# HiLab-git/FPL-plus

Hardware: NVIDIA B200
Metric: train_voxels_per_s (higher is better)
Workload: dtype bf16

## Files before the change

fpl-plus_b200/csrc/convt_tc.cu:

```cuda
#include "common.cuh"
#include "tc_ptx.cuh"
#include "../../include/fplplus_b200.h"

namespace {

constexpr int kTH = 16, kTW = 8;
constexpr int kPlane = kTH * kTW * 16;
constexpr int kThreadsT = 192;
constexpr int kMaxStagesT = 8;

__device__ __forceinline__ void tma_load_4d(void* dst, const CUtensorMap* map, uint64_t* bar, int c0, int c1, int c2, int c3) {
    asm volatile(
        "cp.async.bulk.tensor.4d.shared::cluster.global.tile.mbarrier::complete_tx::bytes [%0], [%1, {%3, %4, %5, %6}], [%2];"
        ::"r"(smem_u32(dst)), "l"(map), "r"(smem_u32(bar)), "r"(c0), "r"(c1), "r"(c2), "r"(c3)
        : "memory");
}

struct CtParams {
    const __nv_bfloat16* image;
    const float* bias;
    bf16x8* out;
    int out_c8tot, out_c8off;
    int a_c8tot, a_c8off;
    int N, D, H, W;
// ... 202 lines not shown
        int ci, co, tap;
        if (mode == 0) { ci = k; tap = nn / cout; co = nn - tap * cout; }
        else { tap = k / cout; co = k - tap * cout; ci = nn; }
        image[i] = __float2bfloat16_rn(w[((int64_t)ci * cout + co) * ntaps + tap]);
    }
}

CUresult encode_4d(EncodeTiledFn encode, CUtensorMap* map, const void* base, int64_t planes, int h, int w, int box_c8,
                   int stride) {
    cuuint64_t gdim[4] = {8, (cuuint64_t)w, (cuuint64_t)h, (cuuint64_t)planes};
    cuuint64_t gstr[3] = {16, (cuuint64_t)w * 16, (cuuint64_t)h * w * 16};
    cuuint32_t box[4] = {8, (cuuint32_t)(kTW * stride), (cuuint32_t)(kTH * stride), (cuuint32_t)box_c8};
    cuuint32_t estr[4] = {1, (cuuint32_t)stride, (cuuint32_t)stride, 1};
    return encode(map, CU_TENSOR_MAP_DATA_TYPE_BFLOAT16, 4, const_cast<void*>(base), gdim, gstr, box, estr,
                  CU_TENSOR_MAP_INTERLEAVE_NONE, CU_TENSOR_MAP_SWIZZLE_NONE, CU_TENSOR_MAP_L2_PROMOTION_L2_128B,
                  CU_TENSOR_MAP_FLOAT_OOB_FILL_NONE);
}

struct CtwParams {
    float* dw;
    int N, D, H, W, cin, cout, kd2, ntaps;
    int x_c8tot, x_c8off, dy_c8tot, dy_c8off;
    int mgroups, m, nb, mtiles, nchunks;
    int x_bytes, dy_tile_bytes, stage_bytes, stages, tmem_cols;
    int tiles_h, tiles_w, tiles_total, split;
    int tapmajor;
};

__global__ void __launch_bounds__(kThreadsT) convt_wgrad_tc_kernel(const __grid_constant__ CUtensorMap xmap,
                                                                  const __grid_constant__ CUtensorMap dymap, CtwParams P) {
    extern __shared__ uint8_t smem_raw[];
    uint8_t* smem = reinterpret_cast<uint8_t*>((reinterpret_cast<uintptr_t>(smem_raw) + 1023) & ~uintptr_t(1023));
    uint64_t* bars = reinterpret_cast<uint64_t*>(smem);
    uint64_t* full_bar = bars;
    uint64_t* empty_bar = bars + kMaxStagesT;
    uint64_t* done_bar = bars + 2 * kMaxStagesT;
    uint32_t* tmem_slot = reinterpret_cast<uint32_t*>(bars + 2 * kMaxStagesT + 1);
    uint8_t* ring = smem + 256;

    const int warp = threadIdx.x >> 5, lane = threadIdx.x & 31;
    int b = blockIdx.x;
    const int slice = b % P.split; b /= P.split;
    const int nc = b % P.nchunks;
    const int mt = b / P.nchunks;
    const int tile_begin = (int)(((int64_t)P.tiles_total * slice) / P.split);
    const int tile_end = (int)(((int64_t)P.tiles_total * (slice + 1)) / P.split);
    const int Do = P.D * P.kd2;

    if (warp == 0 && lane == 0) {
        asm volatile("prefetch.tensormap [%0];" ::"l"(&xmap) : "memory");
        asm volatile("prefetch.tensormap [%0];" ::"l"(&dymap) : "memory");
        for (int s = 0; s < P.stages; ++s) { mbar_init(&full_bar[s], 1); mbar_init(&empty_bar[s], 1); }
        mbar_init(done_bar, 1);
        fence_barrier_init();
    }
    if (warp == 1) tmem_alloc(tmem_slot, (uint32_t)P.tmem_cols);
    FPL_PDL_WAIT();
    tc_fence_before();
    __syncthreads();
    tc_fence_after();
    const uint32_t tmem_base = *tmem_slot;

    if (warp == 0) {
        if (lane == 0) {
            int stage = 0; uint32_t phase = 0;
            for (int t = tile_begin; t < tile_end; ++t) {
                int r = t;
                const int tw = r % P.tiles_w; r /= P.tiles_w;
                const int th = r % P.tiles_h; r /= P.tiles_h;
                const int d = r % P.D;
                const int n = r / P.D;
                mbar_wait(&empty_bar[stage], phase ^ 1);
                uint8_t* x_dst = ring + (size_t)stage * P.stage_bytes;
                mbar_expect_tx(&full_bar[stage], (uint32_t)(P.x_bytes + P.ntaps * P.dy_tile_bytes));
                tma_load_4d(x_dst, &xmap, &full_bar[stage], 0, tw * kTW, th * kTH,
                            (n * P.D + d) * P.x_c8tot + P.x_c8off + mt * P.mgroups);
                for (int tap = 0; tap < P.ntaps; ++tap) {
                    const int a = P.kd2 == 2 ? tap >> 2 : 0, bb = (tap >> 1) & 1, c = tap & 1;
                    tma_load_4d(x_dst + P.x_bytes + (size_t)tap * P.dy_tile_bytes, &dymap, &full_bar[stage], 0,
                                2 * tw * kTW + c, 2 * th * kTH + bb,
                                (n * Do + d * P.kd2 + a) * P.dy_c8tot + P.dy_c8off + nc * (P.nb / 8));
                }
                if (++stage == P.stages) { stage = 0; phase ^= 1; }
            }
        }
    } else if (warp == 1) {
        const uint32_t idesc = (1u << 4) | (1u << 7) | (1u << 10) | (1u << 15) | (1u << 16) |
                               ((uint32_t)(P.nb >> 3) << 17) | ((uint32_t)(P.m >> 4) << 24);
        const uint64_t hi = make_desc(0, kTW * 16, kPlane);
        const uint32_t ring_u = smem_u32(ring);
        const bool leader = elect_one();
        int stage = 0; uint32_t phase = 0;
        uint32_t accumulate = 0;
        for (int t = tile_begin; t < tile_end; ++t) {
            mbar_wait(&full_bar[stage], phase);
            tc_fence_after();
            const uint32_t x_base = (ring_u + (uint32_t)stage * (uint32_t)P.stage_bytes) >> 4;
            const uint32_t dy_base = x_base + ((uint32_t)P.x_bytes >> 4);
            uint64_t adesc = hi + (uint64_t)x_base, b_hp = hi + (uint64_t)dy_base;
            const uint64_t dy_tile16 = (uint64_t)((uint32_t)P.dy_tile_bytes >> 4);
            for (int hp = 0; hp < kTH / 2; ++hp, adesc += 2 * kTW * 16 / 16, b_hp += 2 * kTW * 16 / 16) {
                uint64_t bdesc = b_hp;
                uint32_t d_tap = tmem_base;
                for (int tap = 0; tap < P.ntaps; ++tap, bdesc += dy_tile16, d_tap += (uint32_t)P.nb) {
                    if (leader) umma_bf16(d_tap, adesc, bdesc, idesc, accumulate);
                }
                accumulate = 1;
            }
            if (leader) umma_commit(&empty_bar[stage]);
            __syncwarp();
            if (++stage == P.stages) { stage = 0; phase ^= 1; }
        }
        if (leader) umma_commit(done_bar);
        __syncwarp();
        FPL_PDL_TRIGGER();
    } else if (tile_end > tile_begin) {
        const int quarter = warp & 3;
        mbar_wait(done_bar, 0);
        tc_fence_after();
        const int tlane = quarter * 32 + lane;
        int row = P.m == 128 ? tlane : ((lane < 16) ? quarter * 16 + lane : -1);
        const bool valid = row >= 0 && row < P.mgroups * 8 && (mt * P.mgroups * 8 + row) < P.cin;
        const int ci = mt * P.mgroups * 8 + row;
        for (int tap = 0; tap < P.ntaps; ++tap) {
            for (int c0 = 0; c0 < P.nb; c0 += 16) {
                uint32_t r[16];
                tmem_ld16(tmem_base + ((uint32_t)(quarter * 32) << 16) + (uint32_t)(tap * P.nb + c0), r);
                tmem_ld_wait();
                if (valid) {
#pragma unroll
                    for (int i = 0; i < 16; ++i) {
                        const int co = nc * P.nb + c0 + i;
                        if (P.tapmajor) atomicAdd(P.dw + ((int64_t)tap * P.cout + co) * P.cin + ci, __uint_as_float(r[i]));
                        else atomicAdd(P.dw + ((int64_t)ci * P.cout + co) * P.ntaps + tap, __uint_as_float(r[i]));
                    }
                }
            }
        }
    }
    tc_fence_before();
    __syncthreads();
    if (warp == 1) {
        tc_fence_after();
        tmem_dealloc(tmem_base, (uint32_t)P.tmem_cols);
    }
}

}

extern "C" int64_t fpl_convt_weight_image_bytes(int cin, int cout, int kd2) {
    return (int64_t)cin * cout * 4 * kd2 * 2;
}

extern "C" int fpl_convt_prep_weight(const float* w, int cin, int cout, int kd2, int mode, void* image, void* stream) {
    FPL_REQUIRE(kd2 == 1 || kd2 == 2, "fpl_convt_prep_weight: kd2=%d must be 1 or 2", kd2);
    const int ntaps = 4 * kd2;
    CtCfg c;
    const int kdim = mode == 0 ? cin : ntaps * cout, ndim = mode == 0 ? ntaps * cout : cin;
    FPL_REQUIRE(make_ct_cfg(kdim, ndim, mode == 0 ? cin : cout, c), "fpl_convt_prep_weight: unsupported channels (%d -> %d)", cin, cout);
    const int total = kdim * ndim;
    int blocks = (total + 255) / 256;
    if (blocks > FPL_NUM_SMS * 4) blocks = FPL_NUM_SMS * 4;
    fpl_launch(convt_prep_kernel, blocks, 256, 0, (cudaStream_t)stream, w, (__nv_bfloat16*)image, cin, cout, ntaps, mode, c.nb, c.kc,
                                                               c.nchunks, total);
    FPL_LAUNCH_CHECK();
    return 0;
}

// ... 75 lines not shown
    int64_t total = (int64_t)P.tiles_h * P.tiles_w * d * n * c.nslices;
    FPL_REQUIRE(total < (1ll << 30), "fpl_convt_k2s2_tc: too many tiles");
    P.total_items = (int)total;
    FPL_CHECK_CUDA(cudaFuncSetAttribute(convt_gemm_tc_kernel, cudaFuncAttributeMaxDynamicSharedMemorySize, c.smem_bytes));
    int grid = FPL_NUM_SMS * 2;
    if (grid > P.total_items) grid = P.total_items;
    fpl_launch(convt_gemm_tc_kernel, grid, kThreadsT, c.smem_bytes, (cudaStream_t)stream, amap, P);
    FPL_LAUNCH_CHECK();
    return 0;
}

extern "C" int fpl_convt_k2s2_fwd_tc(const void* x, int x_c8tot, int x_c8off, const void* image, const float* bias, void* y,
                                     int y_c8tot, int y_c8off, int n, int d, int h, int w, int cin, int cout, int kd2,
                                     void* stream) {
    return convt_gemm_launch(0, x, x_c8tot, x_c8off, image, bias, y, y_c8tot, y_c8off, n, d, h, w, cin, cout, kd2, stream);
}

extern "C" int fpl_convt_k2s2_dgrad_tc(const void* dy, int dy_c8tot, int dy_c8off, const void* image_t, void* dx, int dx_c8tot,
                                       int dx_c8off, int n, int d, int h, int w, int cin, int cout, int kd2, void* stream) {
    return convt_gemm_launch(1, dy, dy_c8tot, dy_c8off, image_t, nullptr, dx, dx_c8tot, dx_c8off, n, d, h, w, cin, cout, kd2,
                             stream);
}

static int convt_wgrad_launch(const void* x, int x_c8tot, int x_c8off, const void* dy, int dy_c8tot, int dy_c8off,
                              float* dw, int n, int d, int h, int w, int cin, int cout, int kd2, void* stream, int tapmajor) {
    FPL_REQUIRE(kd2 == 1 || kd2 == 2, "fpl_convt_k2s2_wgrad_tc: kd2=%d must be 1 or 2", kd2);
    FPL_REQUIRE(cin % 8 == 0 && cout % 16 == 0, "fpl_convt_k2s2_wgrad_tc: unsupported channels (%d -> %d)", cin, cout);
    EncodeTiledFn encode = get_encode_fn();
    FPL_REQUIRE(encode != nullptr, "fpl_convt_k2s2_wgrad_tc: cuTensorMapEncodeTiled not available from the driver");
    CtwParams P;
    P.dw = dw; P.N = n; P.D = d; P.H = h; P.W = w; P.cin = cin; P.cout = cout; P.kd2 = kd2; P.ntaps = 4 * kd2;
    P.x_c8tot = x_c8tot; P.x_c8off = x_c8off; P.dy_c8tot = dy_c8tot; P.dy_c8off = dy_c8off; P.tapmajor = tapmajor;
    const int g_all = cin / 8;
    P.mgroups = g_all < 16 ? g_all : 16;
    FPL_REQUIRE(g_all % P.mgroups == 0, "fpl_convt_k2s2_wgrad_tc: cin=%d not tileable", cin);
    P.mtiles = g_all / P.mgroups;
    P.m = P.mgroups <= 8 ? 64 : 128;
    P.nb = cout % 32 == 0 ? 32 : 16;
    P.x_bytes = P.mgroups * kPlane;
    if (2 * (P.x_bytes + P.ntaps * (P.nb / 8) * kPlane) > 200 * 1024 - (P.m / 8) * kPlane) P.nb = 16;
    P.nchunks = cout / P.nb;
    P.dy_tile_bytes = (P.nb / 8) * kPlane;
    P.stage_bytes = P.x_bytes + P.ntaps * P.dy_tile_bytes;
    P.stages = (200 * 1024 - (P.m / 8) * kPlane) / P.stage_bytes;
    if (P.stages > kMaxStagesT) P.stages = kMaxStagesT;
    FPL_REQUIRE(P.stages >= 2, "fpl_convt_k2s2_wgrad_tc: stage of %d bytes does not fit twice", P.stage_bytes);
    int cols = P.ntaps * P.nb;
    P.tmem_cols = 32;
    while (P.tmem_cols < cols) P.tmem_cols *= 2;
    CUtensorMap xmap, dymap;
    CUresult r = encode_4d(encode, &xmap, x, (int64_t)n * d * x_c8tot, h, w, P.mgroups, 1);
    FPL_REQUIRE(r == CUDA_SUCCESS, "fpl_convt_k2s2_wgrad_tc: tensor map (x) failed (%d)", (int)r);
    r = encode_4d(encode, &dymap, dy, (int64_t)n * d * kd2 * dy_c8tot, 2 * h, 2 * w, P.nb / 8, 2);
    FPL_REQUIRE(r == CUDA_SUCCESS, "fpl_convt_k2s2_wgrad_tc: tensor map (dy) failed (%d)", (int)r);
    P.tiles_h = (h + kTH - 1) / kTH; P.tiles_w = (w + kTW - 1) / kTW;
    int64_t tiles = (int64_t)P.tiles_h * P.tiles_w * d * n;
    FPL_REQUIRE(tiles < (1ll << 30), "fpl_convt_k2s2_wgrad_tc: too many tiles");
    P.tiles_total = (int)tiles;
    const int pairs = P.mtiles * P.nchunks;
    int split = FPL_NUM_SMS / pairs;
    if (split > P.tiles_total / 4) split = P.tiles_total / 4;
    if (split < 1) split = 1;
    P.split = split;
    const int smem_bytes = P.stages * P.stage_bytes + (P.m / 8) * kPlane + 1024 + 256;
    FPL_CHECK_CUDA(cudaFuncSetAttribute(convt_wgrad_tc_kernel, cudaFuncAttributeMaxDynamicSharedMemorySize, smem_bytes));
    fpl_launch(convt_wgrad_tc_kernel, pairs * split, kThreadsT, smem_bytes, (cudaStream_t)stream, xmap, dymap, P);
    FPL_LAUNCH_CHECK();
    return 0;
}

extern "C" int fpl_convt_k2s2_wgrad_tc(const void* x, int x_c8tot, int x_c8off, const void* dy, int dy_c8tot, int dy_c8off,
                                       float* dw, int n, int d, int h, int w, int cin, int cout, int kd2, void* stream) {
    return convt_wgrad_launch(x, x_c8tot, x_c8off, dy, dy_c8tot, dy_c8off, dw, n, d, h, w, cin, cout, kd2, stream, 0);
}

extern "C" int fpl_convt_k2s2_wgrad_tc_tapmajor(const void* x, int x_c8tot, int x_c8off, const void* dy, int dy_c8tot,
                                                int dy_c8off, float* scratch, int n, int d, int h, int w, int cin, int cout,
                                                int kd2, void* stream) {
    return convt_wgrad_launch(x, x_c8tot, x_c8off, dy, dy_c8tot, dy_c8off, scratch, n, d, h, w, cin, cout, kd2, stream, 1);
}
```

fpl-plus_b200/lib.py:

```python
import ctypes
from ctypes import c_char_p, c_double, c_float, c_int, c_int64, c_longlong, c_uint64, c_void_p

from . import build as _build

_P = c_void_p
_I = c_int
_L = c_int64
_F = c_float
_U = c_uint64

_SIGNATURES = {
    "fpl_last_error": (c_char_p, []),
    "fpl_version": (_I, []),
    "fpl_set_sm_budget": (_I, [_I]),
    "fpl_launch_count": (c_longlong, [_I]),
    "fpl_device_is_sm100": (_I, []),
    "fpl_conv3d_weight_image_bytes": (_L, [_I, _I, _I]),
    "fpl_conv3d_prep_weight": (_I, [_P, _I, _I, _I, _I, _P, _P]),
    "fpl_conv3d_prep_weight_batch": (_I, [_I, ctypes.POINTER(c_void_p), ctypes.POINTER(_I), ctypes.POINTER(_I),
                                          ctypes.POINTER(_I), ctypes.POINTER(_I), ctypes.POINTER(c_void_p), _P]),
    "fpl_conv3d_tc": (_I, [_P, _I, _I, _P, _P, _P, _I, _I, _P] + [_I] * 7 + [_P]),
    "fpl_conv3d_dfold_image_bytes": (_L, [_I, _I]),
    "fpl_conv3d_dfold_prep_weight": (_I, [_P, _I, _I, _I, _P, _P]),
    "fpl_conv3d_dfold_prep_weight_batch": (_I, [_I, ctypes.POINTER(c_void_p), ctypes.POINTER(_I), ctypes.POINTER(_I),
# ... 16 lines not shown
    "fpl_maxpool_c8": (_I, [_P, _I, _I, _P, _I, _I, _I] + [_I] * 5 + [_P]),
    "fpl_head_fwd": (_I, [_P, _I, _I, _P, _P, _P] + [_I] * 6 + [_P]),
    "fpl_head_dgrad": (_I, [_P, _P, _P, _I, _I, _P, _I, _I, _P] + [_I] * 6 + [_P]),
    "fpl_upsample2x_c8": (_I, [_P, _I, _I, _P, _I, _I] + [_I] * 6 + [_P]),
    "fpl_upsample2x_c8_bwd": (_I, [_P, _I, _I, _P, _I, _I] + [_I] * 6 + [_P]),
    "fpl_channel_sum_c8": (_I, [_P, _I, _I, _P] + [_I] * 5 + [_P]),
    "fpl_grad_scatter_add": (_I, [_P, _P, _P, _I, _I, _P]),
    "fpl_stem_conv_fwd": (_I, [_P, _P, _P, _P, _I, _I, _P] + [_I] * 7 + [_P]),
    "fpl_stem_conv_wgrad": (_I, [_P, _P, _I, _I, _P] + [_I] * 7 + [_P]),
    "fpl_head_conv_fwd": (_I, [_P, _I, _I, _P, _P, _P] + [_I] * 6 + [_P]),
    "fpl_head_conv_tc": (_I, [_P, _I, _I, _P, _P, _P] + [_I] * 6 + [_P]),
    "fpl_pack_ncdhw_to_c8": (_I, [_P, _I, _P, _I, _I, _I, _P] + [_I] * 4 + [_P]),
    "fpl_head_conv_bwd": (_I, [_P, _I, _I, _P, _P, _P, _I, _I, _P, _P] + [_I] * 6 + [_P]),
    "fpl_convt_k2s2_fwd": (_I, [_P, _I, _I, _P, _P, _P, _I, _I] + [_I] * 7 + [_P]),
    "fpl_convt_k2s2_bwd": (_I, [_P, _I, _I, _P, _P, _I, _I, _P, _I, _I, _P, _P] + [_I] * 7 + [_P]),
    "fpl_convt_weight_image_bytes": (_L, [_I, _I, _I]),
    "fpl_convt_prep_weight": (_I, [_P, _I, _I, _I, _I, _P, _P]),
    "fpl_convt_prep_weight_batch": (_I, [_I, ctypes.POINTER(c_void_p), ctypes.POINTER(_I), ctypes.POINTER(_I),
                                         ctypes.POINTER(_I), ctypes.POINTER(_I), ctypes.POINTER(c_void_p), _P]),
    "fpl_convt_k2s2_fwd_tc": (_I, [_P, _I, _I, _P, _P, _P, _I, _I] + [_I] * 7 + [_P]),
    "fpl_convt_k2s2_dgrad_tc": (_I, [_P, _I, _I, _P, _P, _I, _I] + [_I] * 7 + [_P]),
    "fpl_convt_k2s2_wgrad_tc": (_I, [_P, _I, _I, _P, _I, _I, _P] + [_I] * 7 + [_P]),
    "fpl_convt_k2s2_wgrad_tc_tapmajor": (_I, [_P, _I, _I, _P, _I, _I, _P] + [_I] * 7 + [_P]),
    "fpl_dsbn_finalize": (_I, [_P, _L, _P, _P, _P, _P, _P, _F, _F, _I, _P, _P, _P, _P, _I, _P]),
    "fpl_dsbn_act_fwd": (_I, [_P, _P, _P, _P, _P, _I, _I, _P, _I, _I, _P, _I, _F, _P, _U, _U, _P] + [_I] * 5 + [_P]),
    "fpl_dsbn_bn_act_fwd": (_I, [_P, _P, _L, _P, _P, _P, _P, _P, _F, _F, _I, _P, _P, _P, _P, _P,
                                 _P, _I, _I, _P, _I, _I, _P, _I, _F, _P, _U, _U, _P] + [_I] * 5 + [_P]),
    "fpl_dsbn_act_bwd_apply_fin": (_I, [_P, _P, _I, _I, _P, _I, _I, _P, _I, _P, _P, _P, _P, _P, _F, _P, _U, _U, _P, _P, _I, _P]
                                   + [_I] * 5 + [_P, _P, _P, _P, _P]),
    "fpl_dsbn_act_bwd_reduce": (_I, [_P, _P, _I, _I, _P, _I, _I, _P, _I, _P, _P, _P, _P, _P, _F, _P, _U, _U, _P, _P]
                                + [_I] * 5 + [_P]),
    "fpl_dsbn_act_bwd_apply": (_I, [_P, _P, _I, _I, _P, _I, _I, _P, _I, _P, _P, _P, _P, _P, _F, _P, _U, _U, _P, _P, _I, _P]
                               + [_I] * 5 + [_P]),
    "fpl_dsbn_bwd_finalize": (_I, [_P, _P, _P, _I, _P, _P, _P, _P, _I, _P]),
    "fpl_gather_patches": (_I, [_P, _I, _I, _I, _I, _I, _P, _P, _P, _P]),
    "fpl_gather_patches_norm_workspace_bytes": (_L, [_I] * 5),
    "fpl_gather_patches_norm": (_I, [_P, _I, _I, _I, _I, _I, ctypes.POINTER(_I), ctypes.POINTER(_F), ctypes.POINTER(_F), _P,
                                     _L, _P, _P, _P, _P]),
    "fpl_adam_multi_tensor": (_I, [_P, _I, _P, _I, _P, c_double, c_double, c_double, c_double, c_double, _P, _P]),
    "fpl_adam_chunk_elems": (_I, []),
    "fpl_dice_ce_reduce": (_I, [_P, _P, _P, _P, _I, _I, _L, _P]),
    "fpl_dice_ce_grad": (_I, [_P, _P, _P, _P, _F, _F, _F, _P, _P, _P, _I, _I, _L, _P]),
    "fpl_dice_ce_reduce_ex": (_I, [_P, _P, _P, _P, _P, _P, _P, _I, _I, _L, _I, _I, _P]),
    "fpl_dice_ce_grad_ex": (_I, [_P, _P, _P, _P, _P, _P, _P, _F, _F, _F, _F, _P, _P, _P, _I, _I, _L, _I, _I, _P]),
    "fpl_dice_ce_loss_ex": (_I, [_P, _P, _P, _P, _P, _P, _P, _F, _F, _F, _P, _P, _I, _I, _L, _I, _I, _P]),
    "fpl_argmax_label": (_I, [_P, _P, _I, _I, _L, _P]),
# ... 50 lines not shown
```

fpl-plus_b200/net.py:

```python
import ctypes
import os

import torch
import torch.nn as nn

from . import ops
from .ops import C8, call, ptr, stream_ptr


class DomainSpecificBatchNorm2d(nn.Module):
    def __init__(self, num_features, num_domains):
        super().__init__()
        self.bns = nn.ModuleList([nn.BatchNorm2d(num_features) for _ in range(num_domains)])


class DomainSpecificBatchNorm3d(nn.Module):
    def __init__(self, num_features, num_domains):
        super().__init__()
        self.bns = nn.ModuleList([nn.BatchNorm3d(num_features) for _ in range(num_domains)])


class ConvBlockND(nn.Module):

    def __init__(self, in_channels, out_channels, num_domains=None, dim=2, dropout_p=0.5):
# ... 62 lines not shown

    def c8(self, name, n, d, c, h, w):
        return self.get(name, (n, d, c // 8, h, w, 8), torch.bfloat16)


class _Lease(object):

    def __init__(self, pool, ws):
        self.pool, self.ws = pool, ws

    def __del__(self):
        try:
            self.pool.append(self.ws)
        except Exception:
            pass


class _Plan(object):

    def __init__(self):
        self.fwd, self.dgrad, self.wgrad = {}, {}, {}
        self.head = None
        self.up = []
        self.images = []
        self.eval_fuse = False


class UNet2D5_dsbn(nn.Module):

    def __init__(self, params):
        super().__init__()
        self.params = params
        self.in_chns = params['in_chns']
        self.ft_chns = list(params['feature_chns'])
        self.dropout = list(params['dropout'])
        self.dims = list(params['conv_dims'])
        self.n_class = params['class_num']
        self.bilinear = params['bilinear']
        self.num_domains = params['num_domains']
        assert len(self.ft_chns) == 5
        ft, nd, dm, dp = self.ft_chns, self.num_domains, self.dims, self.dropout
        self.block0 = DownBlock(self.in_chns, ft[0], nd, dm[0], dp[0], True)
        self.block1 = DownBlock(ft[0], ft[1], nd, dm[1], dp[1], True)
        self.block2 = DownBlock(ft[1], ft[2], nd, dm[2], dp[2], True)
        self.block3 = DownBlock(ft[2], ft[3], nd, dm[3], dp[3], True)
        self.block4 = DownBlock(ft[3], ft[4], nd, dm[4], dp[4], False)
# ... 285 lines not shown
        if grad and stem_tc and stem.cout == 16 and w0 >= 32 and h0 >= 4:
            plan.fwd[stem.name] = "stem_direct"
        elif stem_tc and d0 >= 2 and stem.cout in (16, 32, 64):
            plan.fwd[stem.name] = "stem_patch"
            plan.images.append(("stem", stem.conv, 0, 3))
        else:
            plan.fwd[stem.name] = "stem_cc"
        if grad:
            wg = plan.fwd[stem.name]
            if wg == "stem_cc" and tc(16, stem.cout) and stem.cin <= 8:
                wg = "stem_c8"
            plan.wgrad[stem.name] = wg
        units = [(u, geo[i][0]) for i in range(5) for u in self._down_units[i] if not u.is_stem]
        units += [(u, geo[3 - k][0]) for k in range(4) for u in self._up_units[k]]
        for u, depth in units:
            kern = plan.fwd[u.name] = conv(u.cin, u.cout, u.kd, depth)
            if kern != "direct":
                plan.images.append((kern, u.conv, 0, u.kd))
            if grad:
                kern = plan.dgrad[u.name] = conv(u.cout, u.cin, u.kd, depth)
                if kern != "direct":
                    plan.images.append((kern, u.conv, 1, u.kd))
                plan.wgrad[u.name] = "tapmajor" if sm100 and u.cin % 8 == 0 and u.cout % 16 == 0 else "direct"
        for k in range(4):
            c, c_low = ft[3 - k], ft[4 - k]
            if not self.bilinear:
                plan.up.append("tc" if tc(c_low, c) else "direct")
                continue
            if not tc(c_low, c):
                raise NotImplementedError("bilinear=True needs feature_chns that are multiples of 16 (tensor-core 1x1 "
                                          "projection)")
            plan.up.append("proj")
            pu = self._proj_units[k]
            plan.images += [("tc", pu.conv, t, 1) for t in ((0, 1) if grad else (0,))]
        if impl_tc and ft[0] in (16, 32) and k_cls <= 8 and d0 >= 2 and n * d0 <= 65535:
            plan.head = "cc"
        elif tc(ft[0], 16) and k_cls <= 8:
            plan.head = "tc"
        else:
            plan.head = "direct"
        if tc(ft[0], 16) and k_cls <= 8:
            plan.images += [("tc", self._head, t, 1) for t in ((0, 1) if grad else (0,))]
        for up in (self.up1, self.up2, self.up3, self.up4):
            trans = up.trans3d if up.dim == 3 else up.trans2d
            if tc(trans.in_channels, trans.out_channels):
                plan.images += [("convt", trans, t, 2 if up.dim == 3 else 1) for t in ((0, 1) if grad else (0,))]
        return plan

    def prepare(self, shape, grad=False):
        plan = self._plan(shape[0], self._geometry(tuple(shape)), grad, ops.is_sm100())
        lib = ops._lib.load()
        todo = {"dfold": [], "convt": [], "tc": []}
        synced = set()
        for kind, conv, t, kd in plan.images:
            if kind == "stem":
# ... 395 lines not shown
        for k, lvl in zip((3, 2, 1, 0), (0, 1, 2, 3)):
            u1, u2 = self._up_units[k]
            up = ups[k]
            c, c_low = ft[lvl], ft[lvl + 1]
            g = self._unit_bwd(u2, rec[u2.name], g, None, None, 0, n, ws, small, grads, True, fold, plan)
            dcat = self._unit_bwd(u1, rec[u1.name], g, None, None, 0, n, ws, small, grads, True, fold, plan)
            skip_grads[lvl] = C8(dcat.buf, 0, c)
            trans = up.trans3d if up.dim == 3 else up.trans2d
            kd2 = 2 if up.dim == 3 else 1
            dl, hl, wl = geo[lvl + 1]
            low = rec["up%d.low" % (k + 1)]
            glow = C8(ws.c8("dlow%d" % lvl, n, dl, c_low, hl, wl))
            if plan.up[k] == "proj":
                pu = self._proj_units[k]
                proj = up.conv3d if up.dim == 3 else up.conv2d
                g_t = ws.c8("dT:up%d" % (k + 1), n, dl, c, hl, wl)
                call("fpl_upsample2x_c8_bwd", ptr(dcat.buf), 2 * c // 8, c // 8, ptr(g_t), c // 8, 0, n, dl, hl, wl, c, kd2, st)
                call("fpl_channel_sum_c8", ptr(g_t), c // 8, 0, ptr(grads[proj.bias]), n, dl, hl, wl, c, st)
                scr = fold["alloc"](9 * c * c_low)
                call("fpl_conv3d_wgrad_tc_tapmajor", *low.args(), ptr(g_t), c // 8, 0, ptr(scr), n, dl, hl, wl, c_low, c, 1, st)
                fold["pending"].append((scr[4 * c * c_low:5 * c * c_low], grads[proj.weight], c, c_low, 1))
                call("fpl_conv3d_tc", ptr(g_t), c // 8, 0, ptr(self._image("tc", pu.conv, 1)), None, *glow.args(),
                     None, n, dl, hl, wl, c, c_low, 1, st)
            elif plan.up[k] == "tc":
                call("fpl_convt_k2s2_dgrad_tc", ptr(dcat.buf), 2 * c // 8, c // 8, ptr(self._image("convt", trans, 1)),
                     *glow.args(), n, dl, hl, wl, c_low, c, kd2, st)
                scr = fold["alloc"](c_low * c * 4 * kd2)
                call("fpl_convt_k2s2_wgrad_tc_tapmajor", *low.args(), ptr(dcat.buf), 2 * c // 8, c // 8, ptr(scr),
                     n, dl, hl, wl, c_low, c, kd2, st)
                fold["pending"].append((scr, grads[trans.weight], c, c_low, -4 * kd2))
                call("fpl_convt_k2s2_bwd", *low.args(), ptr(trans.weight), ptr(dcat.buf), 2 * c // 8, c // 8, None, 0, 0,
                     None, ptr(grads[trans.bias]), n, dl, hl, wl, c_low, c, kd2, st)
            else:
                call("fpl_convt_k2s2_bwd", *low.args(), ptr(trans.weight), ptr(dcat.buf), 2 * c // 8, c // 8, *glow.args(),
                     ptr(grads[trans.weight]), ptr(grads[trans.bias]), n, dl, hl, wl, c_low, c, kd2, st)
            g = glow
            done += 12
            fire(done)
        g_pool = None
        for i in (4, 3, 2, 1, 0):
            u1, u2 = self._down_units[i]
            r1 = rec[u1.name]
            if i == 4:
                g = self._unit_bwd(u2, rec[u2.name], g, None, None, 0, n, ws, small, grads, True, fold, plan)
            else:
                idx, pool_kd = rec["idx%d" % i]
# ... 104 lines not shown
```

include/fplplus_b200.h:

```cpp
#ifndef FPLPLUS_B200_H
#define FPLPLUS_B200_H

#include <stdint.h>

#ifdef __cplusplus
extern "C" {
#endif

const char* fpl_last_error(void);
int fpl_version(void);
int fpl_set_sm_budget(int sms);
long long fpl_launch_count(int reset);
int fpl_device_is_sm100(void);


int64_t fpl_conv3d_weight_image_bytes(int cin, int cout, int kd);
int fpl_conv3d_prep_weight(const float* w, int cin, int cout, int kd, int transpose_flip,
                           void* image, void* stream);
int fpl_conv3d_prep_weight_batch(int count, const float* const* h_w, const int* h_cin, const int* h_cout,
                                 const int* h_kd, const int* h_transpose_flip, void* const* h_images, void* stream);
int fpl_conv3d_tc(const void* x, int x_c8tot, int x_c8off, const void* image, const float* bias,
                  void* y, int y_c8tot, int y_c8off, double* stats,
                  int n, int d, int h, int w, int cin, int cout, int kd, void* stream);
int64_t fpl_conv3d_dfold_image_bytes(int cin, int cout);
// ... 83 lines not shown
                      void* dx, int dx_c8tot, int dx_c8off, float* dw, float* db,
                      int n, int d, int h, int w_, int cin, int classes, void* stream);

int fpl_convt_k2s2_fwd(const void* x, int x_c8tot, int x_c8off, const float* w, const float* bias,
                       void* y, int y_c8tot, int y_c8off, int n, int d, int h, int w_, int cin, int cout,
                       int kd2, void* stream);
int fpl_convt_k2s2_bwd(const void* x, int x_c8tot, int x_c8off, const float* w,
                       const void* dy, int dy_c8tot, int dy_c8off,
                       void* dx, int dx_c8tot, int dx_c8off, float* dw, float* db,
                       int n, int d, int h, int w_, int cin, int cout, int kd2, void* stream);

int64_t fpl_convt_weight_image_bytes(int cin, int cout, int kd2);
int fpl_convt_prep_weight(const float* w, int cin, int cout, int kd2, int mode, void* image, void* stream);
int fpl_convt_prep_weight_batch(int count, const float* const* h_w, const int* h_cin, const int* h_cout,
                                const int* h_kd2, const int* h_mode, void* const* h_images, void* stream);
int fpl_convt_k2s2_fwd_tc(const void* x, int x_c8tot, int x_c8off, const void* image, const float* bias, void* y,
                          int y_c8tot, int y_c8off, int n, int d, int h, int w, int cin, int cout, int kd2, void* stream);
int fpl_convt_k2s2_dgrad_tc(const void* dy, int dy_c8tot, int dy_c8off, const void* image_t, void* dx, int dx_c8tot,
                            int dx_c8off, int n, int d, int h, int w, int cin, int cout, int kd2, void* stream);
int fpl_convt_k2s2_wgrad_tc(const void* x, int x_c8tot, int x_c8off, const void* dy, int dy_c8tot, int dy_c8off,
                            float* dw, int n, int d, int h, int w, int cin, int cout, int kd2, void* stream);
int fpl_convt_k2s2_wgrad_tc_tapmajor(const void* x, int x_c8tot, int x_c8off, const void* dy, int dy_c8tot, int dy_c8off,
                                     float* scratch, int n, int d, int h, int w, int cin, int cout, int kd2, void* stream);


int fpl_dsbn_finalize(const double* stats, int64_t count, const float* gamma, const float* beta,
                      float* running_mean, float* running_var, int64_t* num_batches_tracked,
                      float momentum, float eps, int training,
                      float* scale, float* shift, float* save_mean, float* save_invstd, int c, void* stream);
int fpl_dsbn_act_fwd(const void* y, const float* scale, const float* shift, const float* slope,
                     void* a, int a_c8tot, int a_c8off,
                     void* pooled, int p_c8tot, int p_c8off, uint8_t* pool_idx, int pool_kd,
                     float drop_p, const uint8_t* drop_mask, uint64_t seed, uint64_t offset, const uint64_t* seed_dev,
                     int n, int d, int h, int w, int c, void* stream);
int fpl_dsbn_bn_act_fwd(const void* y, const double* stats, int64_t count, const float* gamma, const float* beta,
                        float* running_mean, float* running_var, int64_t* num_batches_tracked, float momentum,
                        float eps, int training, float* scale, float* shift, float* save_mean, float* save_invstd,
                        const float* slope, void* a, int a_c8tot, int a_c8off, void* pooled, int p_c8tot, int p_c8off,
                        uint8_t* pool_idx, int pool_kd, float drop_p, const uint8_t* drop_mask, uint64_t seed,
                        uint64_t offset, const uint64_t* seed_dev, int n, int d, int h, int w, int c, void* stream);
int fpl_dsbn_act_bwd_reduce(const void* y, const void* g1, int g1_c8tot, int g1_c8off,
                            const void* g_pool, int gp_c8tot, int gp_c8off, const uint8_t* pool_idx, int pool_kd,
                            const float* scale, const float* shift, const float* save_mean,
                            const float* save_invstd, const float* slope,
                            float drop_p, const uint8_t* drop_mask, uint64_t seed, uint64_t offset,
                            const uint64_t* seed_dev, double* red, int n, int d, int h, int w, int c, void* stream);
// ... 58 lines not shown
```

Before: 1.028 billion.

## Fuse transposed-conv dgrad, wgrad and bias-grad into one tensor-core backward kernel

Adds a fused backward kernel for the k2s2 transposed conv. Each dy tile loaded for wgrad is also reused for the dgrad MMA against a weight image held in shared memory. dx is written from double-buffered TMEM by the epilogue warps. The bias gradient comes from an appended ones row in the x operand. dy is now fetched with one 5D TMA per (h,w) parity instead of one 4D load per tap, and all taps are packed into a single wide MMA. The aim is to avoid reading dy twice and to cut launches, at the cost of a tighter shared-memory/TMEM budget and a more complex producer/consumer schedule.

Result: faster. 1.048 billion, median of 6 (+1.9%).

```diff
diff --git a/fpl-plus_b200/csrc/convt_tc.cu b/fpl-plus_b200/csrc/convt_tc.cu
--- a/fpl-plus_b200/csrc/convt_tc.cu
+++ b/fpl-plus_b200/csrc/convt_tc.cu
@@ -248,11 +248,19 @@
     int N, D, H, W, cin, cout, kd2, ntaps;
     int x_c8tot, x_c8off, dy_c8tot, dy_c8off;
     int mgroups, m, nb, mtiles, nchunks;
-    int x_bytes, dy_tile_bytes, stage_bytes, stages, tmem_cols;
+    int x_bytes, dy_off, dy_tile_bytes, stage_bytes, stages, tmem_cols;
     int tiles_h, tiles_w, tiles_total, split;
     int tapmajor;
+    const void* image;
+    int image_bytes;
+    bf16x8* dx;
+    int dx_c8tot, dx_c8off;
+    float* db;
 };
 
+__device__ __forceinline__ int ct_slot(int tap, int kd2) { return (tap & 3) * kd2 + (kd2 == 2 ? tap >> 2 : 0); }
+
+template <bool kFused>
 __global__ void __launch_bounds__(kThreadsT) convt_wgrad_tc_kernel(const __grid_constant__ CUtensorMap xmap,
                                                                   const __grid_constant__ CUtensorMap dymap, CtwParams P) {
     extern __shared__ uint8_t smem_raw[];
@@ -261,8 +269,12 @@
     uint64_t* full_bar = bars;
     uint64_t* empty_bar = bars + kMaxStagesT;
     uint64_t* done_bar = bars + 2 * kMaxStagesT;
-    uint32_t* tmem_slot = reinterpret_cast<uint32_t*>(bars + 2 * kMaxStagesT + 1);
+    uint64_t* tmem_full = bars + 2 * kMaxStagesT + 1;
+    uint64_t* tmem_empty = bars + 2 * kMaxStagesT + 3;
+    uint64_t* image_bar = bars + 2 * kMaxStagesT + 5;
+    uint32_t* tmem_slot = reinterpret_cast<uint32_t*>(bars + 2 * kMaxStagesT + 6);
     uint8_t* ring = smem + 256;
+    uint8_t* image_sm = ring + (size_t)P.stages * P.stage_bytes;
 
     const int warp = threadIdx.x >> 5, lane = threadIdx.x & 31;
     int b = blockIdx.x;
@@ -272,13 +284,24 @@
     const int tile_begin = (int)(((int64_t)P.tiles_total * slice) / P.split);
     const int tile_end = (int)(((int64_t)P.tiles_total * (slice + 1)) / P.split);
     const int Do = P.D * P.kd2;
+    const int wcols = P.ntaps * P.nb;
 
     if (warp == 0 && lane == 0) {
         asm volatile("prefetch.tensormap [%0];" ::"l"(&xmap) : "memory");
         asm volatile("prefetch.tensormap [%0];" ::"l"(&dymap) : "memory");
         for (int s = 0; s < P.stages; ++s) { mbar_init(&full_bar[s], 1); mbar_init(&empty_bar[s], 1); }
         mbar_init(done_bar, 1);
+        if (kFused) {
+            for (int a = 0; a < 2; ++a) { mbar_init(&tmem_full[a], 1); mbar_init(&tmem_empty[a], 4); }
+            mbar_init(image_bar, 1);
+        }
         fence_barrier_init();
+    }
+    if (kFused) {
+        for (int s = 0; s < P.stages; ++s)
+            for (int i = threadIdx.x; i < kPlane / 4; i += kThreadsT)
+                reinterpret_cast<uint32_t*>(ring + (size_t)s * P.stage_bytes + P.x_bytes)[i] = 0x3F803F80u;
+        fence_proxy_async();
     }
     if (warp == 1) tmem_alloc(tmem_slot, (uint32_t)P.tmem_cols);
     FPL_PDL_WAIT();
@@ -289,6 +312,10 @@
 
     if (warp == 0) {
         if (lane == 0) {
+            if (kFused && tile_end > tile_begin) {
+                mbar_expect_tx(image_bar, (uint32_t)P.image_bytes);
+                bulk_load(image_sm, P.image, (uint32_t)P.image_bytes, image_bar);
+            }
             int stage = 0; uint32_t phase = 0;
             for (int t = tile_begin; t < tile_end; ++t) {
                 int r = t;
@@ -301,37 +328,49 @@
                 mbar_expect_tx(&full_bar[stage], (uint32_t)(P.x_bytes + P.ntaps * P.dy_tile_bytes));
                 tma_load_4d(x_dst, &xmap, &full_bar[stage], 0, tw * kTW, th * kTH,
                             (n * P.D + d) * P.x_c8tot + P.x_c8off + mt * P.mgroups);
-                for (int tap = 0; tap < P.ntaps; ++tap) {
-                    const int a = P.kd2 == 2 ? tap >> 2 : 0, bb = (tap >> 1) & 1, c = tap & 1;
-                    tma_load_4d(x_dst + P.x_bytes + (size_t)tap * P.dy_tile_bytes, &dymap, &full_bar[stage], 0,
-                                2 * tw * kTW + c, 2 * th * kTH + bb,
-                                (n * Do + d * P.kd2 + a) * P.dy_c8tot + P.dy_c8off + nc * (P.nb / 8));
-                }
+                for (int bc = 0; bc < 4; ++bc)
+                    tma_load_5d(x_dst + P.dy_off + (size_t)bc * P.kd2 * P.dy_tile_bytes, &dymap, &full_bar[stage], 0,
+                                2 * tw * kTW + (bc & 1), 2 * th * kTH + (bc >> 1), P.dy_c8off + nc * (P.nb / 8),
+                                n * Do + d * P.kd2);
                 if (++stage == P.stages) { stage = 0; phase ^= 1; }
             }
         }
     } else if (warp == 1) {
         const uint32_t idesc = (1u << 4) | (1u << 7) | (1u << 10) | (1u << 15) | (1u << 16) |
-                               ((uint32_t)(P.nb >> 3) << 17) | ((uint32_t)(P.m >> 4) << 24);
+                               ((uint32_t)(wcols >> 3) << 17) | ((uint32_t)(P.m >> 4) << 24);
         const uint64_t hi = make_desc(0, kTW * 16, kPlane);
+        const uint32_t idesc_dx = (1u << 4) | (1u << 7) | (1u << 10) | ((uint32_t)(P.cin >> 3) << 17) | (8u << 24);
+        const uint64_t a_hi_dx = make_desc(0, kPlane, kTW * 16), b_hi_dx = make_desc(0, (uint32_t)P.cin * 16, 128);
+        const int cg_tap = P.nb / 8;
         const uint32_t ring_u = smem_u32(ring);
         const bool leader = elect_one();
         int stage = 0; uint32_t phase = 0;
+        int acc = 0; uint32_t acc_phase = 0;
         uint32_t accumulate = 0;
+        if (kFused && tile_end > tile_begin) mbar_wait(image_bar, 0);
         for (int t = tile_begin; t < tile_end; ++t) {
             mbar_wait(&full_bar[stage], phase);
             tc_fence_after();
             const uint32_t x_base = (ring_u + (uint32_t)stage * (uint32_t)P.stage_bytes) >> 4;
-            const uint32_t dy_base = x_base + ((uint32_t)P.x_bytes >> 4);
-            uint64_t adesc = hi + (uint64_t)x_base, b_hp = hi + (uint64_t)dy_base;
-            const uint64_t dy_tile16 = (uint64_t)((uint32_t)P.dy_tile_bytes >> 4);
-            for (int hp = 0; hp < kTH / 2; ++hp, adesc += 2 * kTW * 16 / 16, b_hp += 2 * kTW * 16 / 16) {
-                uint64_t bdesc = b_hp;
-                uint32_t d_tap = tmem_base;
-                for (int tap = 0; tap < P.ntaps; ++tap, bdesc += dy_tile16, d_tap += (uint32_t)P.nb) {
-                    if (leader) umma_bf16(d_tap, adesc, bdesc, idesc, accumulate);
+            const uint32_t dy_base = x_base + ((uint32_t)P.dy_off >> 4);
+            uint64_t adesc = hi + (uint64_t)x_base, bdesc = hi + (uint64_t)dy_base;
+            for (int hp = 0; hp < kTH / 2; ++hp, adesc += 2 * kTW * 16 / 16, bdesc += 2 * kTW * 16 / 16) {
+                if (leader) umma_bf16(tmem_base, adesc, bdesc, idesc, accumulate);
+                accumulate = 1;
+            }
+            if (kFused) {
+                mbar_wait(&tmem_empty[acc], acc_phase ^ 1);
+                tc_fence_after();
+                const uint32_t d_tmem = tmem_base + (uint32_t)(wcols + acc * P.cin);
+                const uint64_t b0 = b_hi_dx + (uint64_t)(smem_u32(image_sm) >> 4);
+                const int ksteps = P.ntaps * P.cout / 16;
+                for (int j = 0; j < ksteps; ++j) {
+                    const int tap = (j * 2) / cg_tap, g = j * 2 - tap * cg_tap;
+                    const uint64_t a = a_hi_dx + (uint64_t)(dy_base + (uint32_t)((ct_slot(tap, P.kd2) * cg_tap + g) * (kPlane / 16)));
+                    if (leader) umma_bf16(d_tmem, a, b0 + (uint64_t)(j * 2 * P.cin), idesc_dx, j > 0 ? 1u : 0u);
                 }
-                accumulate = 1;
+                if (leader) umma_commit(&tmem_full[acc]);
+                if (++acc == 2) { acc = 0; acc_phase ^= 1; }
             }
             if (leader) umma_commit(&empty_bar[stage]);
             __syncwarp();
@@ -342,16 +381,55 @@
         FPL_PDL_TRIGGER();
     } else if (tile_end > tile_begin) {
         const int quarter = warp & 3;
+        if (kFused) {
+            const int row = quarter * 32 + lane;
+            const int hl = row / kTW, wl = row % kTW;
+            const int64_t HW = (int64_t)P.H * P.W;
+            int acc = 0; uint32_t acc_phase = 0;
+            for (int t = tile_begin; t < tile_end; ++t) {
+                int r = t;
+                const int tw = r % P.tiles_w; r /= P.tiles_w;
+                const int th = r % P.tiles_h; r /= P.tiles_h;
+                const int d = r % P.D;
+                const int n = r / P.D;
+                mbar_wait(&tmem_full[acc], acc_phase);
+                tc_fence_after();
+                const int h = th * kTH + hl, w = tw * kTW + wl;
+                const bool valid = h < P.H && w < P.W;
+                const uint32_t t_row = tmem_base + ((uint32_t)(quarter * 32) << 16) + (uint32_t)(wcols + acc * P.cin);
+                for (int c0 = 0; c0 < P.cin; c0 += 16) {
+                    uint32_t rr[16];
+                    tmem_ld16(t_row + (uint32_t)c0, rr);
+                    tmem_ld_wait();
+                    float v[16];
+#pragma unroll
+                    for (int i = 0; i < 16; ++i) v[i] = __uint_as_float(rr[i]);
+                    if (valid) {
+                        bf16x8* dst = P.dx + (((int64_t)n * P.D + d) * P.dx_c8tot + P.dx_c8off + c0 / 8) * HW + (int64_t)h * P.W + w;
+                        st_bf16x8(dst, v);
+                        st_bf16x8(dst + HW, v + 8);
+                    }
+                }
+                tc_fence_before();
+                __syncwarp();
+                if (lane == 0) mbar_arrive(&tmem_empty[acc]);
+                if (++acc == 2) { acc = 0; acc_phase ^= 1; }
+            }
+        }
         mbar_wait(done_bar, 0);
         tc_fence_after();
         const int tlane = quarter * 32 + lane;
         int row = P.m == 128 ? tlane : ((lane < 16) ? quarter * 16 + lane : -1);
         const bool valid = row >= 0 && row < P.mgroups * 8 && (mt * P.mgroups * 8 + row) < P.cin;
+        const bool ones_row = kFused && row == P.cin;
         const int ci = mt * P.mgroups * 8 + row;
-        for (int tap = 0; tap < P.ntaps; ++tap) {
-            for (int c0 = 0; c0 < P.nb; c0 += 16) {
+        for (int c0 = 0; c0 < P.nb; c0 += 16) {
+            float bsum[16];
+#pragma unroll
+            for (int i = 0; i < 16; ++i) bsum[i] = 0.0f;
+            for (int tap = 0; tap < P.ntaps; ++tap) {
                 uint32_t r[16];
-                tmem_ld16(tmem_base + ((uint32_t)(quarter * 32) << 16) + (uint32_t)(tap * P.nb + c0), r);
+                tmem_ld16(tmem_base + ((uint32_t)(quarter * 32) << 16) + (uint32_t)(ct_slot(tap, P.kd2) * P.nb + c0), r);
                 tmem_ld_wait();
                 if (valid) {
 #pragma unroll
@@ -361,6 +439,14 @@
                         else atomicAdd(P.dw + ((int64_t)ci * P.cout + co) * P.ntaps + tap, __uint_as_float(r[i]));
                     }
                 }
+                if (ones_row) {
+#pragma unroll
+                    for (int i = 0; i < 16; ++i) bsum[i] += __uint_as_float(r[i]);
+                }
+            }
+            if (ones_row) {
+#pragma unroll
+                for (int i = 0; i < 16; ++i) atomicAdd(P.db + c0 + i, bsum[i]);
             }
         }
     }
@@ -370,6 +456,17 @@
         tc_fence_after();
         tmem_dealloc(tmem_base, (uint32_t)P.tmem_cols);
     }
+}
+
+CUresult encode_dy_5d(EncodeTiledFn encode, CUtensorMap* map, const void* dy, int64_t n_do, int c8tot, int ho, int wo, int box_c8,
+                      int kd2) {
+    cuuint64_t gdim[5] = {8, (cuuint64_t)wo, (cuuint64_t)ho, (cuuint64_t)c8tot, (cuuint64_t)n_do};
+    cuuint64_t gstr[4] = {16, (cuuint64_t)wo * 16, (cuuint64_t)ho * wo * 16, (cuuint64_t)c8tot * ho * wo * 16};
+    cuuint32_t box[5] = {8, (cuuint32_t)(kTW * 2), (cuuint32_t)(kTH * 2), (cuuint32_t)box_c8, (cuuint32_t)kd2};
+    cuuint32_t estr[5] = {1, 2, 2, 1, 1};
+    return encode(map, CU_TENSOR_MAP_DATA_TYPE_BFLOAT16, 5, const_cast<void*>(dy), gdim, gstr, box, estr,
+                  CU_TENSOR_MAP_INTERLEAVE_NONE, CU_TENSOR_MAP_SWIZZLE_NONE, CU_TENSOR_MAP_L2_PROMOTION_L2_128B,
+                  CU_TENSOR_MAP_FLOAT_OOB_FILL_NONE);
 }
 
 }
@@ -491,51 +588,91 @@
                              stream);
 }
 
-static int convt_wgrad_launch(const void* x, int x_c8tot, int x_c8off, const void* dy, int dy_c8tot, int dy_c8off,
-                              float* dw, int n, int d, int h, int w, int cin, int cout, int kd2, void* stream, int tapmajor) {
-    FPL_REQUIRE(kd2 == 1 || kd2 == 2, "fpl_convt_k2s2_wgrad_tc: kd2=%d must be 1 or 2", kd2);
-    FPL_REQUIRE(cin % 8 == 0 && cout % 16 == 0, "fpl_convt_k2s2_wgrad_tc: unsupported channels (%d -> %d)", cin, cout);
-    EncodeTiledFn encode = get_encode_fn();
-    FPL_REQUIRE(encode != nullptr, "fpl_convt_k2s2_wgrad_tc: cuTensorMapEncodeTiled not available from the driver");
-    CtwParams P;
-    P.dw = dw; P.N = n; P.D = d; P.H = h; P.W = w; P.cin = cin; P.cout = cout; P.kd2 = kd2; P.ntaps = 4 * kd2;
-    P.x_c8tot = x_c8tot; P.x_c8off = x_c8off; P.dy_c8tot = dy_c8tot; P.dy_c8off = dy_c8off; P.tapmajor = tapmajor;
+namespace {
+constexpr int kWgSmemBudget = 200 * 1024;
+
+bool make_ctw_cfg(int cin, int cout, int kd2, bool fused, CtwParams& P, int& smem_bytes) {
+    if (!(kd2 == 1 || kd2 == 2) || cin % 8 || cout % 16) return false;
+    P.cin = cin; P.cout = cout; P.kd2 = kd2; P.ntaps = 4 * kd2;
     const int g_all = cin / 8;
     P.mgroups = g_all < 16 ? g_all : 16;
-    FPL_REQUIRE(g_all % P.mgroups == 0, "fpl_convt_k2s2_wgrad_tc: cin=%d not tileable", cin);
+    if (g_all % P.mgroups) return false;
     P.mtiles = g_all / P.mgroups;
-    P.m = P.mgroups <= 8 ? 64 : 128;
-    P.nb = cout % 32 == 0 ? 32 : 16;
+    const int mrows = fused ? cin + 8 : P.mgroups * 8;
+    P.m = mrows <= 64 ? 64 : 128;
     P.x_bytes = P.mgroups * kPlane;
-    if (2 * (P.x_bytes + P.ntaps * (P.nb / 8) * kPlane) > 200 * 1024 - (P.m / 8) * kPlane) P.nb = 16;
+    P.dy_off = P.x_bytes + (fused ? kPlane : 0);
+    P.image_bytes = 0;
+    int slack = (P.m / 8) * kPlane;
+    if (fused) {
+        if (mrows > 128 || cin % 16 || P.ntaps * cout > 256 || P.ntaps * cout + 2 * cin > 512) return false;
+        P.nb = cout;
+        P.image_bytes = P.ntaps * cout * cin * 2;
+        slack = 0;
+    } else {
+        P.nb = cout % 32 == 0 ? 32 : 16;
+        if (2 * (P.x_bytes + P.ntaps * (P.nb / 8) * kPlane) > kWgSmemBudget - slack) P.nb = 16;
+    }
     P.nchunks = cout / P.nb;
     P.dy_tile_bytes = (P.nb / 8) * kPlane;
-    P.stage_bytes = P.x_bytes + P.ntaps * P.dy_tile_bytes;
-    P.stages = (200 * 1024 - (P.m / 8) * kPlane) / P.stage_bytes;
+    P.stage_bytes = P.dy_off + P.ntaps * P.dy_tile_bytes;
+    P.stages = (kWgSmemBudget - slack - P.image_bytes) / P.stage_bytes;
     if (P.stages > kMaxStagesT) P.stages = kMaxStagesT;
-    FPL_REQUIRE(P.stages >= 2, "fpl_convt_k2s2_wgrad_tc: stage of %d bytes does not fit twice", P.stage_bytes);
-    int cols = P.ntaps * P.nb;
+    if (P.stages < 2) return false;
+    const int cols = P.ntaps * P.nb + (fused ? 2 * cin : 0);
     P.tmem_cols = 32;
     while (P.tmem_cols < cols) P.tmem_cols *= 2;
+    smem_bytes = P.stages * P.stage_bytes + slack + P.image_bytes + 1024 + 256;
+    return true;
+}
+
+int convt_wgrad_launch(const void* x, int x_c8tot, int x_c8off, const void* dy, int dy_c8tot, int dy_c8off, float* dw, int n,
+                       int d, int h, int w, int cin, int cout, int kd2, void* stream, int tapmajor, const void* image = nullptr,
+                       void* dx = nullptr, int dx_c8tot = 0, int dx_c8off = 0, float* db = nullptr) {
+    const bool fused = image != nullptr;
+    const char* name = fused ? "fpl_convt_k2s2_bwd_tc" : "fpl_convt_k2s2_wgrad_tc";
+    FPL_REQUIRE(kd2 == 1 || kd2 == 2, "%s: kd2=%d must be 1 or 2", name, kd2);
+    FPL_REQUIRE(cin % 8 == 0 && cout % 16 == 0, "%s: unsupported channels (%d -> %d)", name, cin, cout);
+    CtwParams P;
+    int smem_bytes = 0;
+    FPL_REQUIRE(make_ctw_cfg(cin, cout, kd2, fused, P, smem_bytes), "%s: channels %d -> %d (kd2 %d) do not fit", name, cin, cout,
+                kd2);
+    FPL_REQUIRE(P.ntaps * P.nb <= 256 && P.m <= 128, "%s: MMA shape M=%d N=%d", name, P.m, P.ntaps * P.nb);
+    FPL_REQUIRE(P.tmem_cols <= 512, "%s: %d TMEM columns", name, P.tmem_cols);
+    FPL_REQUIRE(smem_bytes <= 227 * 1024, "%s: %d bytes of shared memory", name, smem_bytes);
+    FPL_REQUIRE(P.tmem_cols <= 256 || 2 * smem_bytes > 228 * 1024, "%s: %d TMEM columns with %d bytes of shared memory",
+                name, P.tmem_cols, smem_bytes);
+    if (fused) {
+        FPL_REQUIRE(dx != nullptr && db != nullptr && P.mtiles == 1 && P.nchunks == 1, "%s: bad arguments", name);
+        CtCfg c;
+        FPL_REQUIRE(make_ct_cfg(P.ntaps * cout, cin, cout, c) && c.nslices == 1 && c.nb == cin &&
+                    c.nchunks * c.b_bytes == P.image_bytes, "%s: dgrad image layout", name);
+    }
+    EncodeTiledFn encode = get_encode_fn();
+    FPL_REQUIRE(encode != nullptr, "%s: cuTensorMapEncodeTiled not available from the driver", name);
+    P.dw = dw; P.N = n; P.D = d; P.H = h; P.W = w;
+    P.x_c8tot = x_c8tot; P.x_c8off = x_c8off; P.dy_c8tot = dy_c8tot; P.dy_c8off = dy_c8off; P.tapmajor = tapmajor;
+    P.image = image; P.dx = (bf16x8*)dx; P.dx_c8tot = dx_c8tot; P.dx_c8off = dx_c8off; P.db = db;
     CUtensorMap xmap, dymap;
     CUresult r = encode_4d(encode, &xmap, x, (int64_t)n * d * x_c8tot, h, w, P.mgroups, 1);
-    FPL_REQUIRE(r == CUDA_SUCCESS, "fpl_convt_k2s2_wgrad_tc: tensor map (x) failed (%d)", (int)r);
-    r = encode_4d(encode, &dymap, dy, (int64_t)n * d * kd2 * dy_c8tot, 2 * h, 2 * w, P.nb / 8, 2);
-    FPL_REQUIRE(r == CUDA_SUCCESS, "fpl_convt_k2s2_wgrad_tc: tensor map (dy) failed (%d)", (int)r);
+    FPL_REQUIRE(r == CUDA_SUCCESS, "%s: tensor map (x) failed (%d)", name, (int)r);
+    r = encode_dy_5d(encode, &dymap, dy, (int64_t)n * d * kd2, dy_c8tot, 2 * h, 2 * w, P.nb / 8, kd2);
+    FPL_REQUIRE(r == CUDA_SUCCESS, "%s: tensor map (dy) failed (%d)", name, (int)r);
     P.tiles_h = (h + kTH - 1) / kTH; P.tiles_w = (w + kTW - 1) / kTW;
     int64_t tiles = (int64_t)P.tiles_h * P.tiles_w * d * n;
-    FPL_REQUIRE(tiles < (1ll << 30), "fpl_convt_k2s2_wgrad_tc: too many tiles");
+    FPL_REQUIRE(tiles < (1ll << 30), "%s: too many tiles", name);
     P.tiles_total = (int)tiles;
     const int pairs = P.mtiles * P.nchunks;
     int split = FPL_NUM_SMS / pairs;
     if (split > P.tiles_total / 4) split = P.tiles_total / 4;
     if (split < 1) split = 1;
     P.split = split;
-    const int smem_bytes = P.stages * P.stage_bytes + (P.m / 8) * kPlane + 1024 + 256;
-    FPL_CHECK_CUDA(cudaFuncSetAttribute(convt_wgrad_tc_kernel, cudaFuncAttributeMaxDynamicSharedMemorySize, smem_bytes));
-    fpl_launch(convt_wgrad_tc_kernel, pairs * split, kThreadsT, smem_bytes, (cudaStream_t)stream, xmap, dymap, P);
+    auto kernel = fused ? convt_wgrad_tc_kernel<true> : convt_wgrad_tc_kernel<false>;
+    FPL_CHECK_CUDA(cudaFuncSetAttribute(kernel, cudaFuncAttributeMaxDynamicSharedMemorySize, smem_bytes));
+    fpl_launch(kernel, pairs * split, kThreadsT, smem_bytes, (cudaStream_t)stream, xmap, dymap, P);
     FPL_LAUNCH_CHECK();
     return 0;
+}
 }
 
 extern "C" int fpl_convt_k2s2_wgrad_tc(const void* x, int x_c8tot, int x_c8off, const void* dy, int dy_c8tot, int dy_c8off,
@@ -548,3 +685,18 @@
                                                 int kd2, void* stream) {
     return convt_wgrad_launch(x, x_c8tot, x_c8off, dy, dy_c8tot, dy_c8off, scratch, n, d, h, w, cin, cout, kd2, stream, 1);
 }
+
+extern "C" int fpl_convt_k2s2_bwd_tc_supported(int cin, int cout, int kd2) {
+    CtwParams P;
+    int smem_bytes = 0;
+    return make_ctw_cfg(cin, cout, kd2, true, P, smem_bytes) && smem_bytes <= 227 * 1024 &&
+           (P.tmem_cols <= 256 || 2 * smem_bytes > 228 * 1024) ? 1 : 0;
+}
+
+extern "C" int fpl_convt_k2s2_bwd_tc(const void* x, int x_c8tot, int x_c8off, const void* dy, int dy_c8tot, int dy_c8off,
+                                     const void* image_t, void* dx, int dx_c8tot, int dx_c8off, float* scratch, float* db, int n,
+                                     int d, int h, int w, int cin, int cout, int kd2, void* stream) {
+    FPL_REQUIRE(image_t != nullptr, "fpl_convt_k2s2_bwd_tc: no dgrad image");
+    return convt_wgrad_launch(x, x_c8tot, x_c8off, dy, dy_c8tot, dy_c8off, scratch, n, d, h, w, cin, cout, kd2, stream, 1,
+                              image_t, dx, dx_c8tot, dx_c8off, db);
+}
diff --git a/fpl-plus_b200/lib.py b/fpl-plus_b200/lib.py
--- a/fpl-plus_b200/lib.py
+++ b/fpl-plus_b200/lib.py
@@ -62,6 +62,8 @@
     "fpl_convt_k2s2_dgrad_tc": (_I, [_P, _I, _I, _P, _P, _I, _I] + [_I] * 7 + [_P]),
     "fpl_convt_k2s2_wgrad_tc": (_I, [_P, _I, _I, _P, _I, _I, _P] + [_I] * 7 + [_P]),
     "fpl_convt_k2s2_wgrad_tc_tapmajor": (_I, [_P, _I, _I, _P, _I, _I, _P] + [_I] * 7 + [_P]),
+    "fpl_convt_k2s2_bwd_tc_supported": (_I, [_I, _I, _I]),
+    "fpl_convt_k2s2_bwd_tc": (_I, [_P, _I, _I, _P, _I, _I, _P, _P, _I, _I, _P, _P] + [_I] * 7 + [_P]),
     "fpl_dsbn_finalize": (_I, [_P, _L, _P, _P, _P, _P, _P, _F, _F, _I, _P, _P, _P, _P, _I, _P]),
     "fpl_dsbn_act_fwd": (_I, [_P, _P, _P, _P, _P, _I, _I, _P, _I, _I, _P, _I, _F, _P, _U, _U, _P] + [_I] * 5 + [_P]),
     "fpl_dsbn_bn_act_fwd": (_I, [_P, _P, _L, _P, _P, _P, _P, _P, _F, _F, _I, _P, _P, _P, _P, _P,
diff --git a/fpl-plus_b200/net.py b/fpl-plus_b200/net.py
--- a/fpl-plus_b200/net.py
+++ b/fpl-plus_b200/net.py
@@ -108,6 +108,7 @@
         self.fwd, self.dgrad, self.wgrad = {}, {}, {}
         self.head = None
         self.up = []
+        self.up_bwd = []
         self.images = []
         self.eval_fuse = False
 
@@ -439,15 +440,20 @@
                 if kern != "direct":
                     plan.images.append((kern, u.conv, 1, u.kd))
                 plan.wgrad[u.name] = "tapmajor" if sm100 and u.cin % 8 == 0 and u.cout % 16 == 0 else "direct"
+        ups = (self.up1, self.up2, self.up3, self.up4)
         for k in range(4):
             c, c_low = ft[3 - k], ft[4 - k]
             if not self.bilinear:
                 plan.up.append("tc" if tc(c_low, c) else "direct")
+                kd2 = 2 if ups[k].dim == 3 else 1
+                fused = plan.up[k] == "tc" and lib.fpl_convt_k2s2_bwd_tc_supported(c_low, c, kd2)
+                plan.up_bwd.append("fused" if fused else plan.up[k])
                 continue
             if not tc(c_low, c):
                 raise NotImplementedError("bilinear=True needs feature_chns that are multiples of 16 (tensor-core 1x1 "
                                           "projection)")
             plan.up.append("proj")
+            plan.up_bwd.append("proj")
             pu = self._proj_units[k]
             plan.images += [("tc", pu.conv, t, 1) for t in ((0, 1) if grad else (0,))]
         if impl_tc and ft[0] in (16, 32) and k_cls <= 8 and d0 >= 2 and n * d0 <= 65535:
@@ -889,6 +895,12 @@
                 fold["pending"].append((scr[4 * c * c_low:5 * c * c_low], grads[proj.weight], c, c_low, 1))
                 call("fpl_conv3d_tc", ptr(g_t), c // 8, 0, ptr(self._image("tc", pu.conv, 1)), None, *glow.args(),
                      None, n, dl, hl, wl, c, c_low, 1, st)
+            elif plan.up_bwd[k] == "fused":
+                scr = fold["alloc"](c_low * c * 4 * kd2)
+                call("fpl_convt_k2s2_bwd_tc", *low.args(), ptr(dcat.buf), 2 * c // 8, c // 8,
+                     ptr(self._image("convt", trans, 1)), *glow.args(), ptr(scr), ptr(grads[trans.bias]),
+                     n, dl, hl, wl, c_low, c, kd2, st)
+                fold["pending"].append((scr, grads[trans.weight], c, c_low, -4 * kd2))
             elif plan.up[k] == "tc":
                 call("fpl_convt_k2s2_dgrad_tc", ptr(dcat.buf), 2 * c // 8, c // 8, ptr(self._image("convt", trans, 1)),
                      *glow.args(), n, dl, hl, wl, c_low, c, kd2, st)
diff --git a/include/fplplus_b200.h b/include/fplplus_b200.h
--- a/include/fplplus_b200.h
+++ b/include/fplplus_b200.h
@@ -129,6 +129,10 @@
                             float* dw, int n, int d, int h, int w, int cin, int cout, int kd2, void* stream);
 int fpl_convt_k2s2_wgrad_tc_tapmajor(const void* x, int x_c8tot, int x_c8off, const void* dy, int dy_c8tot, int dy_c8off,
                                      float* scratch, int n, int d, int h, int w, int cin, int cout, int kd2, void* stream);
+int fpl_convt_k2s2_bwd_tc_supported(int cin, int cout, int kd2);
+int fpl_convt_k2s2_bwd_tc(const void* x, int x_c8tot, int x_c8off, const void* dy, int dy_c8tot, int dy_c8off,
+                          const void* image_t, void* dx, int dx_c8tot, int dx_c8off, float* scratch, float* db, int n, int d,
+                          int h, int w, int cin, int cout, int kd2, void* stream);
 
 
 int fpl_dsbn_finalize(const double* stats, int64_t count, const float* gamma, const float* beta,
```
